# vin2803/scalable-hw-agnostic-inference

Hardware: AMD Instinct MI355X
Metric: SD2.1 512x512 images/sec (50 DDIM steps, CFG 7.5) (higher is better)
Workload: dtype bf16; 1 GPU; model=stabilityai/stable-diffusion-2-1 (UNet2DCondition 865M + OpenCLIP-H text + VAE), global_batch=32, per_gpu_batch=32, seq_len=77, resolution=512x512, inference_steps=50, scheduler=DDIM, parallelism=dp1, hip_graphs=True

## Files before the change

csrc/bindings.cpp:

```cpp
#include <ATen/ATen.h>
#include <c10/hip/HIPStream.h>
#include <torch/library.h>

#include <cmath>
#include <cstdio>
#include <cstdlib>
#include <mutex>
#include <string>
#include <unordered_map>
#include <algorithm>
#include <vector>

#include "kernels/launchers.h"

using at::Tensor;
using c10::optional;

namespace {

#define SHAI_CHECK(cond, ...) TORCH_CHECK(cond, "shai: ", __VA_ARGS__)

hipStream_t stream() { return c10::hip::getCurrentHIPStream().stream(); }

int g_halo_mode = -1;
// ... 1772 lines not shown
  if (bias.has_value()) {
    check_bf16(*bias, "bias");
    SHAI_CHECK(bias->numel() == g.N, "gemm_lnout bias [N]");
    g.bias = cptr(*bias);
  }
  for (const optional<Tensor>* t : {&gamma, &beta})
    if (t->has_value()) {
      check_bf16(**t, "gamma/beta");
      SHAI_CHECK((*t)->numel() == g.N, "gemm_lnout gamma / beta [N]");
    }
  if (!shai::gemm_ws_lnout_supported(g)) return false;
  shai::launch_gemm_ws_lnout(g, mptr(c2), optr(gamma), optr(beta), (float)eps, stream());
  return true;
}

void gemm_f8(const Tensor& a8, const Tensor& w8, const Tensor& a_scale, const Tensor& w_scale, const Tensor& c,
             const optional<Tensor>& bias, const optional<Tensor>& residual, double res_alpha, int64_t act, bool glu,
             int64_t cfg) {
  SHAI_CHECK(a8.is_cuda() && a8.scalar_type() == at::kFloat8_e4m3fn && a8.dim() == 2 && a8.stride(1) == 1,
             "gemm_f8: a8 must be float8_e4m3fn [M, K] with unit column stride");
  SHAI_CHECK(w8.is_cuda() && w8.scalar_type() == at::kFloat8_e4m3fn && w8.dim() == 2 && w8.is_contiguous(),
             "gemm_f8: w8 must be a contiguous float8_e4m3fn [N, K]");
  check_f32(a_scale, "a_scale");
  check_f32(w_scale, "w_scale");
  check_bf16(c, "c");
  const long M = a8.size(0), K = a8.size(1), N = w8.size(0);
  SHAI_CHECK(w8.size(1) == K && a_scale.numel() == M && w_scale.numel() == N, "gemm_f8 shapes");
  SHAI_CHECK(c.dim() == 2 && c.size(0) == M && c.size(1) == (glu ? N / 2 : N) && c.stride(1) == 1, "gemm_f8: c shape");
  shai::GemmArgs g{};
  g.M = (int)M;
// ... 67 lines not shown
  m.def("bias_act(Tensor x, Tensor? bias, Tensor? residual, Tensor(a!) out, int act, float alpha) -> ()");
  m.def("rope(Tensor(a!) x, Tensor positions, Tensor cos, Tensor sin, int rot_dim, bool neox) -> ()");
  m.def("rope_pairs(Tensor(a!) x, Tensor cos, Tensor sin) -> ()");
  m.def("sample(Tensor logits, Tensor temps, Tensor top_k, Tensor top_p, Tensor uniforms, Tensor(a!) out) -> ()");
  m.def("rope_qkv_cache(Tensor(a!) qkv, Tensor positions, Tensor cos, Tensor sin, Tensor(b!) k_cache, Tensor(c!) v_cache, Tensor slots, int H, int Hkv, float k_scale=1.0, float v_scale=1.0) -> ()");
  m.def("sched_step(Tensor model_out, Tensor(a!) latents, bool cfg, float guidance, int pred_type, float a_t, float a_prev, float dt) -> ()");
  m.def("sched_step_rows(Tensor model_out, Tensor(a!) latents, bool cfg, float guidance, int pred_type, Tensor rows_params) -> ()");
  m.def("softmax_(Tensor(a!) x, float scale) -> ()");
  m.def("embedding(Tensor ids, Tensor table, Tensor(a!) out) -> ()");
  m.def("token_feedback(Tensor(a!) ids, Tensor rowmap, Tensor prev) -> ()");
  m.def("decode_attn_rope(Tensor qkv, Tensor(a!) k_cache, Tensor(b!) v_cache, Tensor(c!) o, Tensor block_table, "
        "Tensor ctx_lens, Tensor positions, Tensor cos, Tensor sin, Tensor slots, Tensor(d!) ws, int h, int hk, "
        "int num_splits, float scale, Tensor? qkv_ws=None, int qkv_kg=0, int qkv_k=0, float qkv_eps=-1.0, float k_scale=1.0, float v_scale=1.0) -> ()");
  m.def("gemm_partials(Tensor a, Tensor w, float rms_eps) -> Tensor");
  m.def("gemm_lnout(Tensor a, Tensor w, Tensor(a!) c, Tensor(b!) c2, Tensor? bias, Tensor residual, float res_alpha, Tensor? gamma, Tensor? beta, float eps, int res_rows=0) -> bool");
  m.def("gemm_tuning() -> str[]", &gemm_tuning);
  m.def("gemm_tuning_export() -> str[]", &gemm_tuning_export);
  m.def("gemm_tuning_import(str[] entries) -> int", &gemm_tuning_import);
  m.def("set_halo_conv(int mode, int waves=-1) -> int", &set_halo_conv);
  m.def("set_flash128x2(int mode) -> int", [](int64_t mode) -> int64_t { return shai::set_flash128x2((int)mode); });
  m.def("set_decode_wb(int mode) -> int", [](int64_t mode) -> int64_t { return shai::set_decode_wb((int)mode); });
}

TORCH_LIBRARY_IMPL(shai, CUDA, m) {
  m.impl("rmsnorm", &rmsnorm);
  m.impl("layernorm", &layernorm);
  m.impl("groupnorm_stats", &groupnorm_stats);
  m.impl("groupnorm_from_partials", &groupnorm_from_partials);
  m.impl("col_partials", &col_partials);
  m.impl("row_moments", &row_moments);
  m.impl("groupnorm_apply", &groupnorm_apply);
  m.impl("gemm", &gemm);
  m.impl("dequant_fp8", &dequant_fp8);
  m.impl("dequant_mxfp4", &dequant_mxfp4);
  m.impl("gemm_f8", &gemm_f8);
  m.impl("gemm_lnout", &gemm_lnout);
  m.impl("quant_rows_fp8", &quant_rows_fp8);
  m.impl("layernorm_mod", &layernorm_mod);
  m.impl("qk_norm_rope", &qk_norm_rope);
  m.impl("conv2d", &conv2d);
  m.impl("flash_attn", &flash_attn);
  m.impl("paged_attn_varlen", &paged_attn_varlen);
  m.impl("decode_attn", &decode_attn);
  m.impl("kv_write", &kv_write);
  m.impl("kv_dequant_blocks", &kv_dequant_blocks);
  m.impl("gated_act", &gated_act);
  m.impl("bias_act", &bias_act);
  m.impl("rope", &rope);
  m.impl("rope_pairs", &rope_pairs);
  m.impl("sample", &sample);
  m.impl("rope_qkv_cache", &rope_qkv_cache);
// ... 9 lines not shown
```

csrc/build.py:

```python
#!/usr/bin/env python3
from __future__ import annotations

import argparse
import os
import shutil
import subprocess
import sys
import sysconfig

ROOT = os.path.dirname(os.path.dirname(os.path.abspath(__file__)))
CSRC = os.path.join(ROOT, "csrc")
PKG = os.path.join(ROOT, "scalable-hw-agnostic-inference_amd")
OUT = os.path.join(PKG, "_native")
BUILD = os.path.join(ROOT, "build", "native")
OUT_DEBUG = os.path.join(PKG, "_native_debug")
BUILD_DEBUG = os.path.join(ROOT, "build", "native_debug")
ARCH = os.environ.get("PYTORCH_ROCM_ARCH", "gfx950")
ROCM = os.environ.get("ROCM_PATH", "/opt/rocm")

KERNEL_SRCS = ["kernels/norm.hip", "kernels/gemm.hip", "kernels/gemm_lds.hip", "kernels/gemm_8ph.hip", "kernels/gemm_w4.hip", "kernels/gemm_ws.hip", "kernels/conv_halo.hip", "kernels/attention.hip", "kernels/attention2.hip", "kernels/attention3.hip", "kernels/elementwise.hip", "kernels/dit.hip",
               "kernels/sampling.hip", "kernels/gemv.hip", "kernels/gemv2.hip", "kernels/gemv_fp4.hip",
               "kernels/gemm_f8.hip", "kernels/attention_kv8.hip", "kernels/gemm_fp4.hip"]
NO_SCRATCH = {"kernels/attention.hip": "decode_attn_kernelINS_5KvFp8",
              "kernels/attention_kv8.hip": "flash_fwd_kernelINS_5KvFp8",
              "kernels/gemm_fp4.hip": "gemm_fp4_kernel"}
EXTRA_KFLAGS = {"kernels/attention3.hip": "-mllvm -amdgpu-mfma-vgpr-form -fno-slp-vectorize",
                "kernels/attention2.hip": "-mllvm -amdgpu-mfma-vgpr-form -fno-slp-vectorize",
                "kernels/gemm_w4.hip": "-mllvm -pragma-unroll-threshold=100000",
                "kernels/gemm_ws.hip": "-mllvm -pragma-unroll-threshold=100000 -fno-slp-vectorize",
                "kernels/conv_halo.hip": "-mllvm -pragma-unroll-threshold=100000 -fno-slp-vectorize"}
BINDING_SRCS = ["bindings.cpp", "test_probes.cpp"]
RUNTIME_SRCS = ["runtime/block_manager.cpp", "runtime/scheduler.cpp"]
COMM_SRCS = ["comm/p2p_allreduce.hip"]


def torch_paths():
    import torch
    from torch.utils import cpp_extension as ce
    inc = ce.include_paths(device_type="cuda") if "device_type" in ce.include_paths.__code__.co_varnames else ce.include_paths(True)
    lib = os.path.join(os.path.dirname(torch.__file__), "lib")
    abi = int(torch._C._GLIBCXX_USE_CXX11_ABI)
    return inc, lib, abi


def write_ninja(path: str, out: str = OUT, build_dir: str = BUILD, debug: bool = False) -> dict:
# ... 157 lines not shown
```

csrc/kernels/launchers.h:

```cpp
#pragma once
#include <hip/hip_runtime.h>
#include <stdint.h>

namespace shai {
typedef uint16_t bf16_t;

struct RowNormArgs {
  const bf16_t* x;
  const bf16_t* residual;
  const bf16_t* w;
  const bf16_t* b;
  bf16_t* out;
  bf16_t* residual_out;
  int rows, D;
  long x_stride, out_stride;
  float eps;
  float w_offset;
  int rows_per_w;
  long w_stride;
};
void launch_rmsnorm(const RowNormArgs& a, hipStream_t s);
void launch_layernorm(const RowNormArgs& a, hipStream_t s);

struct GroupNormArgs {
// ... 104 lines not shown
void launch_gemm(const GemmArgs& a, hipStream_t s);
void launch_gemm2(const GemmArgs& a, float* ws, hipStream_t s);
size_t gemm2_workspace_bytes(const GemmArgs& a);
void gemm2_plan(const GemmArgs& a, int* cfg, int* splits);
void launch_gemm2_cfg(const GemmArgs& a, float* ws, int cfg, int splits, hipStream_t s);
int gemm2_num_cfgs();
bool gemm2_cfg_supported(const GemmArgs& a, int cfg);
bool gemm2_cfg_splittable(int cfg);
bool gemm_w4_supported(const GemmArgs& a);
void launch_gemm_w4(const GemmArgs& a, int bn, hipStream_t s);
bool gemm_ws_supported(const GemmArgs& a);
void launch_gemm_ws(const GemmArgs& a, hipStream_t s);
bool gemm_ws_lnout_supported(const GemmArgs& a);
void launch_gemm_ws_lnout(const GemmArgs& a, bf16_t* C2, const bf16_t* gamma, const bf16_t* beta, float eps,
                          hipStream_t s);
bool conv_halo_supported(const GemmArgs& a);
void launch_conv_halo(const GemmArgs& a, hipStream_t s, int waves);
bool gemm2_cfg_candidate(int cfg);
void launch_splitk_epilogue(const GemmArgs& a, const float* ws, int splits, hipStream_t s);
bool gemm4_supported(const GemmArgs& a);
bool gemm4_stats_ok(const GemmArgs& a, int bn);
void launch_gemm4(const GemmArgs& a, float* ws, int splits, int bn, hipStream_t s, bool persist = false);
bool skinny_supported(const GemmArgs& a);
int skinny_kgroups(const GemmArgs& a);
int skinny_max_kgroups(const GemmArgs& a);
size_t skinny_workspace_bytes(const GemmArgs& a);
size_t skinny_workspace_bytes_kg(const GemmArgs& a, int kg);
void launch_skinny(const GemmArgs& a, float* ws, hipStream_t s);
void launch_skinny_kg(const GemmArgs& a, float* ws, int kg, hipStream_t s, bool fixup = false, bool fold = true);
unsigned* skinny_ticket_slice(hipStream_t s, int ntiles);
// ... 101 lines not shown
```

scalable-hw-agnostic-inference_amd/models/unet2d.py:

```python
from __future__ import annotations

import os
from dataclasses import dataclass, field
from typing import List, Optional, Tuple

import torch
import torch.nn as nn

from .. import ops
from .attention import CrossAttention, FusedSelfAttention, merge_linear_keys
from .layers import Conv2d, GLULinear, GroupNorm, LayerNorm, Linear, _wkey, timestep_embedding

MERGE_PROJ_OUT = os.environ.get("SHAI_MERGE_PROJ_OUT", "1") != "0"
GN_FOLD_PROJ_IN = os.environ.get("SHAI_GN_FOLD_PROJ_IN", "1") != "0"

NORM_HANDOFF = os.environ.get("SHAI_NORM_HANDOFF", "1") != "0"
FUSED_GN_CONV = os.environ.get("SHAI_FUSED_GN_CONV", "1") != "0"
CFG_SHARED = os.environ.get("SHAI_CFG_SHARED", "1") != "0"
CFG_SHARED_MIN_ROWS = int(os.environ.get("SHAI_CFG_SHARED_MIN_ROWS", "8192"))


@dataclass
class UNetConfig:
    in_channels: int = 4
# ... 73 lines not shown
class BasicTransformerBlock(nn.Module):
    def __init__(self, dim: int, heads: int, ctx_dim: int):
        super().__init__()
        self.norm1 = LayerNorm(dim)
        self.attn1 = FusedSelfAttention(dim, heads, qkv_bias=False)
        self.norm2 = LayerNorm(dim)
        self.attn2 = CrossAttention(dim, ctx_dim, heads)
        self.norm3 = LayerNorm(dim)
        self.ff = FeedForward(dim)

    def forward(self, x, ctx_kv, shared: bool = False):
        x = self.attn1(self.norm1(x), residual=x)
        x = self.attn2(self.norm2(x), ctx_kv, residual=x, shared=shared)
        return self.ff(self.norm3(x), residual=x)

    def forward_folded(self, x, ctx_kv, mr, next_eps=None, defer_down: bool = False, shared: bool = False):
        B, T, C = x.shape
        a1 = self.attn1
        w, b, s = a1.qkv.folded(self.norm1)
        q, k, v = a1.split(ops.linear(x, w, b, row_affine=(mr, s)))
        o = ops.attention(q, k, v)
        a2 = self.attn2
        H, hd = a2.heads, a2.head_dim
        lnout = x.is_cuda and ops.lnout_supported(B * T, C, a1.heads * a1.head_dim)
        if lnout:
            n2, n3 = self.norm2, self.norm3
            x, xn = ops.linear_lnout(o.view(B, T, a1.heads * a1.head_dim), a1.out.weight, a1.out.bias, x, n2.weight,
                                     n2.bias, n2.eps)
            q = a2.q(xn).view(B, T, H, hd)
        else:
            x, mr = a1.out.forward_stats(o.view(B, T, a1.heads * a1.head_dim), residual=x, stats="ln",
                                         eps=self.norm2.eps)
            w, b, s = a2.q.folded(self.norm2)
            q = ops.linear(x, w, b, row_affine=(mr, s)).view(B, T, H, hd)
        S = ctx_kv.shape[1]
        o = ops.attention(q, ctx_kv[..., : H * hd].view(ctx_kv.shape[0], S, H, hd),
                          ctx_kv[..., H * hd:].view(ctx_kv.shape[0], S, H, hd), q_batch_mod=B if shared else 0)
        rr = B * T if shared else 0
        B = o.shape[0]
        proj = self.ff.net[0].proj
        if lnout:
            x, xn = ops.linear_lnout(o.view(B, T, H * hd), a2.out.weight, a2.out.bias, x, self.norm3.weight,
                                     self.norm3.bias, self.norm3.eps, residual_rows=rr)
            h = ops.linear(xn, proj.weight, proj.bias, act=proj.act, glu=True)
        else:
            x, mr = a2.out.forward_stats(o.view(B, T, H * hd), residual=x, stats="ln", eps=self.norm3.eps,
                                         residual_rows=rr)
            w, b, s = proj.folded(self.norm3)
            h = ops.linear(x, w, b, act=proj.act, glu=True, row_affine=(mr, s))
        if defer_down:
            return h, x
        down = self.ff.net[2]
        if next_eps is None:
            return down(h, residual=x), None
        return down.forward_stats(h, residual=x, stats="ln", eps=next_eps)


class Transformer2DModel(nn.Module):
# ... 15 lines not shown
    def forward_parts(self, x, ctx_kv, xp=None, stats: bool = False, shared: bool = False):
        B, H, W, C = x.shape
        rr = B * H * W if shared else 0
        blocks = list(self.transformer_blocks)
        if ops.fold_profitable(B * H * W, C):
            if self._gn_fold_ok(x):
                h, mr = self._proj_in_gn_folded(x, xp, blocks[0].norm1.eps)
            else:
                h, mr = self.proj_in(self.norm(x, part=xp), stats="ln", eps=blocks[0].norm1.eps)
            h = h.view(B, H * W, C)
            if mr is None:
                mr = ops.row_moments(h, blocks[0].norm1.eps)
            merged = self._merged_out(x.is_cuda)
            for i, blk in enumerate(blocks):
                if i + 1 == len(blocks) and merged is not None:
                    ffh, hx = blk.forward_folded(h, ctx_kv, mr, None, defer_down=True, shared=shared and i == 0)
                    return self._out_merged(ffh, hx, x, merged, stats, rr)
                h, mr = blk.forward_folded(h, ctx_kv, mr, blocks[i + 1].norm1.eps if i + 1 < len(blocks) else None,
                                           shared=shared and i == 0)
        else:
            h = self.proj_in(self.norm(x, part=xp)).view(B, H * W, C)
            for i, blk in enumerate(blocks):
                h = blk(h, ctx_kv, shared=shared and i == 0)
        res = x.view(B, H * W, C)
        B = h.shape[0]
        if stats and ops.stats_supported(B * H * W, C, "gn", H * W):
            out, op = self.proj_out.forward_stats(h, residual=res, stats="gn", residual_rows=rr)
            return out.view(B, H, W, C), op
        return self.proj_out(h, residual=res, residual_rows=rr).view(B, H, W, C), None

    def _gn_fold_ok(self, x) -> bool:
# ... 16 lines not shown
        if down.in_features % 64 or po.in_features % 64:
            return None
        key = tuple(_wkey(t) for t in (down.weight, down.bias, po.weight, po.bias))
        cached = getattr(self, "_po_merged", None)
        if cached is None or cached[0] != key:
            if cuda and torch.cuda.is_current_stream_capturing():
                return None
            wpo = po.weight.float()
            w = torch.cat([wpo @ down.weight.float(), wpo], 1).to(po.weight.dtype).contiguous()
            b = po.bias.float() if po.bias is not None else torch.zeros(po.out_features, device=wpo.device)
            if down.bias is not None:
                b = b + wpo @ down.bias.float()
            cached = (key, (w, b.to(po.weight.dtype)))
            self._po_merged = cached
        return cached[1]

    def _out_merged(self, ffh, hx, x, merged, stats, residual_rows: int = 0):
        _, H, W, C = x.shape
        B = hx.shape[0]
        w, b = merged
        f = ffh.reshape(B, H, W, ffh.shape[-1])
        kw = {"stats": "gn"} if stats and ops.stats_supported(B * H * W, C, "gn", H * W) else {}
        r = ops.conv2d(f, w, b, 1, 1, x2=hx.reshape(B, H, W, C), residual=x, residual_rows=residual_rows, **kw)
        return r if kw else (r, None)


class Downsample2D(nn.Module):
    def __init__(self, ch):
        super().__init__()
        self.conv = Conv2d(ch, ch, 3, stride=2, padding=1)
# ... 195 lines not shown
```

scalable-hw-agnostic-inference_amd/ops/__init__.py:

```python
from __future__ import annotations

import math
import os
from dataclasses import dataclass
from typing import List, Optional, Sequence, Tuple

import torch

from .. import native
from . import reference as ref
from .reference import (ACT_GELU, ACT_GELU_TANH, ACT_NONE, ACT_QUICK_GELU, ACT_RELU, ACT_SILU, act_id, mxfp4_pack,
                        mxfp4_unpack, quantize_mxfp4, pack_conv_weight, pack_up2_phase_weight, unpack_conv_weight)

__all__ = [
    "rmsnorm", "layernorm", "groupnorm_stats", "groupnorm_apply", "groupnorm", "linear", "conv2d", "attention",
    "paged_attention", "decode_attention", "kv_write", "rope", "rope_pairs", "gated_act", "bias_act", "sched_step",
    "softmax_", "embedding", "token_feedback", "decode_attention_rope", "decode_attention_rope_qkv", "gemm_partials", "quantize_fp8_rows", "dequant_fp8", "quantize_mxfp4", "dequant_mxfp4", "mxfp4_pack", "mxfp4_unpack", "is_mxfp4", "quant_rows_fp8", "gemm_f8", "pack_conv_weight", "pack_up2_phase_weight", "linear_wslices", "unpack_conv_weight", "act_id", "ACT_NONE", "ACT_SILU", "ACT_GELU",
    "ACT_GELU_TANH", "ACT_QUICK_GELU", "ACT_RELU", "decode_splits", "set_decode_wb",
    "paged_attention_varlen", "rope_qkv_cache", "quantize_kv_fp8", "dequant_kv_fp8", "kv_dequant_blocks",
    "plan_kv_scratch", "build_kv_rounds", "KVRound", "FP8_KV_DTYPE", "resolve_kv_prefill", "KV_PREFILL_ROUTES",
]


def _gpu(t: torch.Tensor) -> bool:
    return t.is_cuda


def _K():
    return native.ops()


def _i32(t: Optional[torch.Tensor]):
# ... 271 lines not shown
    x2 = x.reshape(-1, K) if (x.dim() == 2 or x.is_contiguous()) else x.contiguous().reshape(-1, K)
    r2 = residual.reshape(-1, N)
    y = torch.empty(x2.shape[0], N, dtype=x.dtype, device=x.device)
    y2 = torch.empty_like(y)
    if LNOUT and _K().gemm_lnout(x2, w, y, y2, bias, r2, 1.0, gamma, beta, float(eps), int(residual_rows)):
        return y.view(*x.shape[:-1], N), y2.view(*x.shape[:-1], N)
    y = linear(x, w, bias, residual=residual, residual_rows=residual_rows)
    return y, layernorm(y, gamma, beta, eps)[0]


LNOUT = os.environ.get("SHAI_LNOUT", "1") != "0"


def lnout_supported(rows: int, n: int, k: int) -> bool:
    return LNOUT and n == 320 and k == 320


def fold_layernorm(w: torch.Tensor, bias: Optional[torch.Tensor], gamma: Optional[torch.Tensor],
                   beta: Optional[torch.Tensor]):
    wf = w.float()
    w2 = (wf * gamma.float()[None, :]).to(w.dtype) if gamma is not None else w
    b2 = bias.float() if bias is not None else torch.zeros(w.shape[0], dtype=torch.float32, device=w.device)
    if beta is not None:
        b2 = b2 + wf @ beta.float()
    return w2.contiguous(), b2.to(w.dtype), w2.float().sum(1).contiguous()


def row_moments(x: torch.Tensor, eps: float) -> torch.Tensor:
    x2 = x.reshape(-1, x.shape[-1])
    if not _gpu(x):
# ... 516 lines not shown
```

scalable-hw-agnostic-inference_amd/ops/reference.py:

```python
from __future__ import annotations

import math

import torch
import torch.nn.functional as F

ACT_NONE, ACT_SILU, ACT_GELU, ACT_GELU_TANH, ACT_QUICK_GELU, ACT_RELU = range(6)
ACT_IDS = {"none": ACT_NONE, None: ACT_NONE, "silu": ACT_SILU, "gelu": ACT_GELU, "gelu_tanh": ACT_GELU_TANH,
           "gelu_pytorch_tanh": ACT_GELU_TANH, "gelu_new": ACT_GELU_TANH, "quick_gelu": ACT_QUICK_GELU,
           "relu": ACT_RELU, "swish": ACT_SILU}


def act_id(act) -> int:
    if isinstance(act, int):
        return act
    return ACT_IDS[act]


def apply_act(x: torch.Tensor, act) -> torch.Tensor:
    a = act_id(act)
    if a == ACT_SILU:
        return F.silu(x)
    if a == ACT_GELU:
        return F.gelu(x)
# ... 100 lines not shown
        y = (mr[:, 1:2] * (y2 - mr[:, 0:1] * s.float()[None, :])).reshape(y.shape)
    y = y * alpha
    if bias is not None:
        y = y + bias.float()
    if glu:
        val, gate = y[..., 0::2], y[..., 1::2]
        y = val * apply_act(gate, act)
    else:
        y = apply_act(y, act)
    if residual is not None:
        r = residual.float()
        if residual_rows:
            r = wrap_rows(r, y.numel() // y.shape[-1], y.shape[-1]).reshape(y.shape)
        y = y + res_alpha * r
    return y.to(x.dtype)


MXFP4_GROUP = 32
MXFP4_VALUES = (0.0, 0.5, 1.0, 1.5, 2.0, 3.0, 4.0, 6.0)


def mxfp4_pack(codes: torch.Tensor, scale_bytes: torch.Tensor):
    N, K2 = codes.shape
    G = scale_bytes.shape[1]
    assert codes.dtype == torch.uint8 and scale_bytes.dtype == torch.uint8 and scale_bytes.shape[0] == N
    assert K2 * 2 == G * MXFP4_GROUP, "one scale per 32 codes"
    steps = (G + 3) // 4
    sb = torch.full((N, steps * 4), 127, dtype=torch.uint8, device=codes.device)
    sb[:, :G] = scale_bytes
    tiled = sb.view(N, steps, 4).permute(1, 0, 2).contiguous()
# ... 390 lines not shown
```

Baseline: 12.28 images/s.

## Fuse GEGLU feed-forward up-projection with merged down/proj_out GEMM in one kernel

Result: no change. 12.30 images/s (median of 2 runs) (+0.1%).

```diff
diff --git a/csrc/bindings.cpp b/csrc/bindings.cpp
--- a/csrc/bindings.cpp
+++ b/csrc/bindings.cpp
@@ -1810,6 +1810,60 @@
   return true;
 }
 
+bool ff_fused(const Tensor& xn, const Tensor& hx, const Tensor& xres, const Tensor& w1, const optional<Tensor>& b1,
+              const Tensor& wm, const optional<Tensor>& bm, const Tensor& out, const optional<Tensor>& part,
+              int64_t res_rows, int64_t max_wgs) {
+  check_rows(xn, "xn");
+  check_rows(hx, "hx");
+  check_rows(xres, "xres");
+  check_rows(w1, "w1");
+  check_rows(wm, "wm");
+  check_bf16(out, "out");
+  if (xn.dim() != 2 || hx.dim() != 2 || xres.dim() != 2 || w1.dim() != 2 || wm.dim() != 2 || out.dim() != 2)
+    return false;
+  shai::FfArgs g{};
+  g.M = (int)xn.size(0);
+  g.C = (int)xn.size(1);
+  g.F = (int)(w1.size(0) / 2);
+  SHAI_CHECK(w1.size(0) == 2 * (int64_t)g.F && w1.size(1) == g.C && wm.size(0) == g.C && wm.size(1) == g.F + g.C,
+             "ff_fused: weights must be w1 [2F, C] and wm [C, F + C]");
+  SHAI_CHECK(hx.size(0) == g.M && hx.size(1) == g.C && out.size(0) == g.M && out.size(1) == g.C &&
+                 xres.size(1) == g.C && xres.size(0) == (res_rows > 0 ? res_rows : (int64_t)g.M),
+             "ff_fused: activation / output / residual shape mismatch");
+  if (res_rows > 0 && res_rows != g.M) g.res_rows = (int)res_rows;
+  g.xn = cptr(xn);
+  g.hx = cptr(hx);
+  g.xres = cptr(xres);
+  g.W1 = cptr(w1);
+  g.Wm = cptr(wm);
+  g.out = mptr(out);
+  g.ldxn = xn.stride(0);
+  g.ldhx = hx.stride(0);
+  g.ldres = xres.stride(0);
+  g.ldw1 = w1.stride(0);
+  g.ldwm = wm.stride(0);
+  g.ldo = out.stride(0);
+  g.max_wgs = (int)max_wgs;
+  if (b1.has_value()) {
+    check_bf16(*b1, "b1");
+    SHAI_CHECK(b1->numel() == 2 * (int64_t)g.F && b1->is_contiguous(), "ff_fused: b1 [2F]");
+    g.b1 = cptr(*b1);
+  }
+  if (bm.has_value()) {
+    check_bf16(*bm, "bm");
+    SHAI_CHECK(bm->numel() == g.C && bm->is_contiguous(), "ff_fused: bm [C]");
+    g.bm = cptr(*bm);
+  }
+  if (part.has_value()) {
+    check_f32(*part, "part");
+    SHAI_CHECK(part->numel() == (int64_t)((g.M + 127) / 128) * g.C * 2, "ff_fused: part [ceil(M / 128), C, 2]");
+    g.col_part = part->data_ptr<float>();
+  }
+  if (!shai::gemm_ff_supported(g)) return false;
+  shai::launch_gemm_ff(g, stream());
+  return true;
+}
+
 void gemm_f8(const Tensor& a8, const Tensor& w8, const Tensor& a_scale, const Tensor& w_scale, const Tensor& c,
              const optional<Tensor>& bias, const optional<Tensor>& residual, double res_alpha, int64_t act, bool glu,
              int64_t cfg) {
@@ -1907,6 +1961,8 @@
         "int num_splits, float scale, Tensor? qkv_ws=None, int qkv_kg=0, int qkv_k=0, float qkv_eps=-1.0, float k_scale=1.0, float v_scale=1.0) -> ()");
   m.def("gemm_partials(Tensor a, Tensor w, float rms_eps) -> Tensor");
   m.def("gemm_lnout(Tensor a, Tensor w, Tensor(a!) c, Tensor(b!) c2, Tensor? bias, Tensor residual, float res_alpha, Tensor? gamma, Tensor? beta, float eps, int res_rows=0) -> bool");
+  m.def("ff_fused(Tensor xn, Tensor hx, Tensor xres, Tensor w1, Tensor? b1, Tensor wm, Tensor? bm, Tensor(a!) out, Tensor(b!)? part, int res_rows=0, int max_wgs=0) -> bool");
+  m.def("ff_fused_set_ablation(int mode) -> ()", [](int64_t mode) { shai::gemm_ff_set_ablation((int)mode); });
   m.def("gemm_tuning() -> str[]", &gemm_tuning);
   m.def("gemm_tuning_export() -> str[]", &gemm_tuning_export);
   m.def("gemm_tuning_import(str[] entries) -> int", &gemm_tuning_import);
@@ -1928,6 +1984,7 @@
   m.impl("dequant_mxfp4", &dequant_mxfp4);
   m.impl("gemm_f8", &gemm_f8);
   m.impl("gemm_lnout", &gemm_lnout);
+  m.impl("ff_fused", &ff_fused);
   m.impl("quant_rows_fp8", &quant_rows_fp8);
   m.impl("layernorm_mod", &layernorm_mod);
   m.impl("qk_norm_rope", &qk_norm_rope);
diff --git a/csrc/build.py b/csrc/build.py
--- a/csrc/build.py
+++ b/csrc/build.py
@@ -18,17 +18,20 @@
 ARCH = os.environ.get("PYTORCH_ROCM_ARCH", "gfx950")
 ROCM = os.environ.get("ROCM_PATH", "/opt/rocm")
 
-KERNEL_SRCS = ["kernels/norm.hip", "kernels/gemm.hip", "kernels/gemm_lds.hip", "kernels/gemm_8ph.hip", "kernels/gemm_w4.hip", "kernels/gemm_ws.hip", "kernels/conv_halo.hip", "kernels/attention.hip", "kernels/attention2.hip", "kernels/attention3.hip", "kernels/elementwise.hip", "kernels/dit.hip",
+KERNEL_SRCS = ["kernels/norm.hip", "kernels/gemm.hip", "kernels/gemm_lds.hip", "kernels/gemm_8ph.hip", "kernels/gemm_w4.hip", "kernels/gemm_ws.hip", "kernels/gemm_ff.hip", "kernels/conv_halo.hip", "kernels/attention.hip", "kernels/attention2.hip", "kernels/attention3.hip", "kernels/elementwise.hip", "kernels/dit.hip",
                "kernels/sampling.hip", "kernels/gemv.hip", "kernels/gemv2.hip", "kernels/gemv_fp4.hip",
                "kernels/gemm_f8.hip", "kernels/attention_kv8.hip", "kernels/gemm_fp4.hip"]
 NO_SCRATCH = {"kernels/attention.hip": "decode_attn_kernelINS_5KvFp8",
               "kernels/attention_kv8.hip": "flash_fwd_kernelINS_5KvFp8",
-              "kernels/gemm_fp4.hip": "gemm_fp4_kernel"}
+              "kernels/gemm_fp4.hip": "gemm_fp4_kernel",
+              "kernels/gemm_ff.hip": "gemm_ff_kernel"}
 EXTRA_KFLAGS = {"kernels/attention3.hip": "-mllvm -amdgpu-mfma-vgpr-form -fno-slp-vectorize",
                 "kernels/attention2.hip": "-mllvm -amdgpu-mfma-vgpr-form -fno-slp-vectorize",
                 "kernels/gemm_w4.hip": "-mllvm -pragma-unroll-threshold=100000",
                 "kernels/gemm_ws.hip": "-mllvm -pragma-unroll-threshold=100000 -fno-slp-vectorize",
-                "kernels/conv_halo.hip": "-mllvm -pragma-unroll-threshold=100000 -fno-slp-vectorize"}
+                "kernels/conv_halo.hip": "-mllvm -pragma-unroll-threshold=100000 -fno-slp-vectorize",
+                "kernels/gemm_ff.hip": ("-mllvm -pragma-unroll-threshold=100000 -fno-slp-vectorize "
+                                        "-mllvm -amdgpu-mfma-vgpr-form")}
 BINDING_SRCS = ["bindings.cpp", "test_probes.cpp"]
 RUNTIME_SRCS = ["runtime/block_manager.cpp", "runtime/scheduler.cpp"]
 COMM_SRCS = ["comm/p2p_allreduce.hip"]
diff --git a/csrc/kernels/gemm_ff.hip b/csrc/kernels/gemm_ff.hip
--- /dev/null
+++ b/csrc/kernels/gemm_ff.hip
@@ -0,0 +1,466 @@
+#include "common.h"
+#include "launchers.h"
+
+#include <algorithm>
+#include <type_traits>
+
+namespace shai {
+
+typedef __bf16 ffbf16x8 __attribute__((ext_vector_type(8)));
+typedef float fff2 __attribute__((ext_vector_type(2)));
+typedef __bf16 ffbf2 __attribute__((ext_vector_type(2)));
+typedef __attribute__((address_space(3))) void ff_lds_void;
+
+constexpr int FF_C = 320, FF_F = 1280, FF_BM = 128;
+constexpr int FF_HC = 32;
+constexpr int FF_NCH = FF_F / FF_HC;
+constexpr int FF_PIECE = 20480;
+constexpr int FF_RING = 7;
+constexpr int FF_AHEAD = FF_RING - 1;
+constexpr int FF_DMA = 5;
+constexpr int FF_B1 = FF_RING * FF_PIECE;
+constexpr int FF_BMO = FF_B1 + 2 * FF_F * 2;
+constexpr int FF_PART = FF_BMO + FF_C * 4;
+constexpr int FF_LDS = FF_PART + 4 * FF_C * 2 * 4;
+constexpr uint32_t FF_OOB = 0x80000000u;
+constexpr int FF_NLD = 20;
+static_assert(FF_LDS <= 160 * 1024, "LDS");
+
+__device__ __forceinline__ __amdgpu_buffer_rsrc_t ff_rsrc(const void* base, long bytes) {
+  return __builtin_amdgcn_make_buffer_rsrc(const_cast<void*>(base), (short)0, (int)(bytes < 0x7fffffffL ? bytes : 0x7fffffffL),
+                                           0x00020000);
+}
+
+__device__ __forceinline__ uint32_t ff_pk(float a, float b) {
+  const fff2 v = {a, b};
+  return __builtin_bit_cast(uint32_t, __builtin_convertvector(v, ffbf2));
+}
+
+__device__ __forceinline__ float ff_row16_sum(float x) {
+  x += __builtin_bit_cast(float, __builtin_amdgcn_update_dpp(0, __builtin_bit_cast(int, x), 0xB1, 0xf, 0xf, true));
+  x += __builtin_bit_cast(float, __builtin_amdgcn_update_dpp(0, __builtin_bit_cast(int, x), 0x4E, 0xf, 0xf, true));
+  x += __builtin_bit_cast(float, __builtin_amdgcn_update_dpp(0, __builtin_bit_cast(int, x), 0x141, 0xf, 0xf, true));
+  x += __builtin_bit_cast(float, __builtin_amdgcn_update_dpp(0, __builtin_bit_cast(int, x), 0x140, 0xf, 0xf, true));
+  return x;
+}
+
+template <bool STATS, int ABL>
+__global__ void __launch_bounds__(256, 1) gemm_ff_kernel(const FfArgs p) {
+  extern __shared__ __attribute__((aligned(16))) char ff_smem[];
+  bf16_t* s_b1 = reinterpret_cast<bf16_t*>(ff_smem + FF_B1);
+  float* s_bm = reinterpret_cast<float*>(ff_smem + FF_BMO);
+  float* s_part = reinterpret_cast<float*>(ff_smem + FF_PART);
+
+  const int tid = threadIdx.x, lane = tid & 63;
+  const int wid = __builtin_amdgcn_readfirstlane(tid >> 6);
+  const int fr = lane & 15, fq = lane >> 4;
+  const int tiles = (p.M + FF_BM - 1) / FF_BM;
+
+  for (int i = tid; i < 2 * FF_F; i += 256) s_b1[i] = p.b1 ? p.b1[i] : (bf16_t)0;
+  for (int i = tid; i < FF_C; i += 256) s_bm[i] = p.bm ? bf2f(p.bm[i]) : 0.f;
+  __syncthreads();
+
+  const long w1_bytes = (long)2 * FF_F * p.ldw1 * 2, wm_bytes = (long)FF_C * p.ldwm * 2;
+  const long xn_bytes = ((long)(p.M - 1) * p.ldxn + FF_C) * 2, hx_bytes = ((long)(p.M - 1) * p.ldhx + FF_C) * 2;
+  const int rrows = p.res_rows > 0 ? p.res_rows : p.M;
+  const long xr_bytes = ((long)(rrows - 1) * p.ldres + FF_C) * 2;
+  const __amdgpu_buffer_rsrc_t rW1 = ff_rsrc(p.W1, w1_bytes), rWm = ff_rsrc(p.Wm, wm_bytes);
+  const __amdgpu_buffer_rsrc_t rXn = ff_rsrc(p.xn, xn_bytes), rHx = ff_rsrc(p.hx, hx_bytes);
+  const __amdgpu_buffer_rsrc_t rXr = ff_rsrc(p.xres, xr_bytes);
+
+  uint32_t off1l[2];
+#pragma unroll
+  for (int e = 0; e < 2; ++e) {
+    const int Rp = 8 * e + (lane >> 3), r = Rp & 15;
+    off1l[e] = (uint32_t)(((16 * (r >> 2) + (r & 3)) * FF_C + (((lane & 7) ^ ((Rp >> 1) & 7)) << 3)) * 2);
+  }
+  auto off1u = [&](int i) {
+    const int q = wid * FF_DMA + i, kt = q >> 2, b = (q & 3) >> 1;
+    return (uint32_t)((4 * b * FF_C + kt * 64) * 2);
+  };
+  uint32_t offml;
+  {
+    const int r = lane >> 2, sc = (lane & 3) ^ ((-(r >> 2)) & 3);
+    offml = (uint32_t)(((8 * (r >> 2) + (r & 3)) * (FF_F + FF_C) + sc * 8) * 2);
+  }
+  auto offmu = [&](int i) {
+    const int j = wid * FF_DMA + i;
+    return (uint32_t)((32 * (j >> 1) + 4 * (j & 1)) * (FF_F + FF_C) * 2);
+  };
+  struct Piece {
+    bool w1;
+    uint32_t so;
+  };
+  auto piece_w1 = [](int c, int h) { return Piece{true, (uint32_t)(c * 64 + h * 8) * (uint32_t)(FF_C * 2)}; };
+  auto piece_wm = [](int kcol) { return Piece{false, (uint32_t)kcol * 2u}; };
+  auto piece_of = [&](int g, int k) {
+    if (g < FF_NCH) return k < 2 ? piece_w1(g, k) : piece_wm(g >= 1 ? FF_HC * (g - 1) : 0);
+    const int idx = 3 * (g - FF_NCH) + k;
+    return piece_wm(idx == 0 ? FF_HC * (FF_NCH - 1) : idx <= 10 ? FF_F + 32 * (idx - 1) : 0);
+  };
+  auto dma_i = [&](const Piece pc, int slot, int i) {
+    if constexpr ((ABL & 4) != 0) return;
+    SHAI_DASSERT(slot >= 0 && slot < FF_RING && i >= 0 && i < FF_DMA);
+    char* dst = ff_smem + slot * FF_PIECE + (wid * FF_DMA + i) * 1024;
+    if (pc.w1) {
+      const uint32_t so = off1u(i) + pc.so;
+      SHAI_DASSERT_DMA(off1l[(wid * FF_DMA + i) & 1] + so, w1_bytes, FF_OOB);
+      __builtin_amdgcn_raw_ptr_buffer_load_lds(rW1, (ff_lds_void*)dst, 16, off1l[(wid * FF_DMA + i) & 1], so, 0, 0);
+    } else {
+      const uint32_t so = offmu(i) + pc.so;
+      SHAI_DASSERT_DMA(offml + so, wm_bytes, FF_OOB);
+      __builtin_amdgcn_raw_ptr_buffer_load_lds(rWm, (ff_lds_void*)dst, 16, offml, so, 0, 0);
+    }
+  };
+
+  const int w1rd = fr * 128, w1sw = (fr >> 1) & 7;
+  auto w1frag = [&](const char* piece, int b, int s) {
+    return *reinterpret_cast<const ffbf16x8*>(piece + (s >> 1) * 4096 + b * 2048 + w1rd +
+                                              (((4 * (s & 1) + fq) ^ w1sw) << 4));
+  };
+  const int wmrd = fr * 64 + ((fq ^ ((-(fr >> 2)) & 3)) << 4);
+  auto wmfrag = [&](const char* piece, int j) {
+    return *reinterpret_cast<const ffbf16x8*>(piece + j * 1024 + wmrd);
+  };
+
+  auto load_rows = [&](const __amdgpu_buffer_rsrc_t& rs, long ld, long r0, int rows, uint4_ (&x)[2][10], int s0,
+                       int s1) {
+#pragma unroll
+    for (int rb = 0; rb < 2; ++rb) {
+      const long row = r0 + 32 * wid + 16 * rb + fr;
+      const uint32_t off = row < rows ? (uint32_t)((row * ld + 8 * fq) * 2) : FF_OOB;
+#pragma unroll
+      for (int s = 0; s < 10; ++s)
+        if (s >= s0 && s < s1)
+          x[rb][s] = __builtin_bit_cast(uint4_, __builtin_amdgcn_raw_buffer_load_b128(rs, (int)(off + 64u * s), 0, 0));
+    }
+  };
+
+  float4_ out[2][20];
+  uint4_ xf[2][10], hf[2][10], rf[2][10];
+  float4_ accA[2][4], accB[2][4];
+
+  auto gemm1 = [&](const char* piece, int h, float4_ (&acc)[2][4], auto&& pre, auto&& between) {
+    ffbf16x8 w[3][2];
+#pragma unroll
+    for (int s = 0; s < 2; ++s)
+#pragma unroll
+      for (int b = 0; b < 2; ++b) w[s][b] = w1frag(piece, b, s);
+#pragma unroll
+    for (int s = 0; s < 10; ++s) {
+      pre(s);
+      if (s + 2 < 10) {
+#pragma unroll
+        for (int b = 0; b < 2; ++b) w[(s + 2) % 3][b] = w1frag(piece, b, s + 2);
+      }
+      __builtin_amdgcn_sched_barrier(0);
+#pragma unroll
+      for (int b = 0; b < 2; ++b)
+#pragma unroll
+        for (int rb = 0; rb < 2; ++rb)
+          acc[rb][2 * h + b] = __builtin_amdgcn_mfma_f32_16x16x32_bf16(
+              w[s % 3][b], __builtin_bit_cast(ffbf16x8, xf[rb][s]),
+              s == 0 ? float4_{0.f, 0.f, 0.f, 0.f} : acc[rb][2 * h + b], 0, 0, 0);
+      if (between(s)) {
+#pragma unroll
+        for (int i = 0; i < 4; ++i) {
+          __builtin_amdgcn_sched_group_barrier(0x008, 1, 0);
+          __builtin_amdgcn_sched_group_barrier(0x002, 5, 0);
+        }
+      }
+      __builtin_amdgcn_sched_barrier(0);
+    }
+  };
+  auto glu_bias = [&](int c, int u) {
+    const uint2_ b = *reinterpret_cast<const uint2_*>(s_b1 + 64 * c + 16 * fq + 4 * (u & 3));
+    return float4_{bf2f(b[0] & 0xffff), bf2f(b[0] >> 16), bf2f(b[1] & 0xffff), bf2f(b[1] >> 16)};
+  };
+  auto glu_half = [&](const float4_ (&acc)[2][4], const float4_ b, int x, float (&o)[2], uint32_t (&ff)[2][4]) {
+    const int u = x >> 1, e = x & 1, rb = u >> 2, jj = u & 3;
+    const float v = acc[rb][jj][2 * e] + b[2 * e], g = acc[rb][jj][2 * e + 1] + b[2 * e + 1];
+    if constexpr ((ABL & 2) != 0) o[e] = v * g;
+    else o[e] = v * gelu_erf_f(g);
+    if (e == 1) ff[rb][jj] = ff_pk(o[0], o[1]);
+  };
+  auto gemm2 = [&](const char* piece, const ffbf16x8 b0, const ffbf16x8 b1, auto&& pre) {
+    ffbf16x8 w[5];
+#pragma unroll
+    for (int j = 0; j < 4; ++j) w[j] = wmfrag(piece, j);
+#pragma unroll
+    for (int j = 0; j < 20; ++j) {
+      pre(j);
+      if (j + 4 < 20) w[(j + 4) % 5] = wmfrag(piece, j + 4);
+      __builtin_amdgcn_sched_barrier(0);
+      out[0][j] = __builtin_amdgcn_mfma_f32_16x16x32_bf16(w[j % 5], b0, out[0][j], 0, 0, 0);
+      out[1][j] = __builtin_amdgcn_mfma_f32_16x16x32_bf16(w[j % 5], b1, out[1][j], 0, 0, 0);
+    }
+    __builtin_amdgcn_sched_barrier(0);
+  };
+
+  int cs = 0;
+  auto sync = [&](auto extra) {
+    constexpr int N = (FF_AHEAD - 1) * FF_DMA + decltype(extra)::value;
+    if constexpr (SHAI_DEBUG) asm volatile("s_waitcnt vmcnt(0)" ::: "memory");
+    else asm volatile("s_waitcnt vmcnt(%0)" ::"n"(N > 63 ? 63 : N) : "memory");
+    asm volatile("s_waitcnt lgkmcnt(0)" ::: "memory");
+    __builtin_amdgcn_sched_barrier(0);
+    __builtin_amdgcn_s_barrier();
+    __builtin_amdgcn_sched_barrier(0);
+  };
+  auto next_slot = [&]() { cs = cs + 1 == FF_RING ? 0 : cs + 1; };
+  auto prev_slot = [&]() { return cs == 0 ? FF_RING - 1 : cs - 1; };
+  using E0 = std::integral_constant<int, 0>;
+  using E20 = std::integral_constant<int, FF_NLD>;
+  using E40 = std::integral_constant<int, 2 * FF_NLD>;
+
+  auto step_w1 = [&](auto extra, const Piece ahead, int c, int h, float4_ (&accN)[2][4], const float4_ (&accP)[2][4],
+                     bool prev, float4_ (&gb)[2], float (&o)[2], uint32_t (&ff)[2][4]) {
+    sync(extra);
+    const int ps = prev_slot();
+    const char* piece = ff_smem + cs * FF_PIECE;
+    if (prev) gb[0] = glu_bias(c - 1, 4 * h);
+    gemm1(
+        piece, h, accN,
+        [&](int s) {
+          if (s < FF_DMA) dma_i(ahead, ps, s);
+          const int nx = 8 * h + s + 1;
+          if (prev && s + 1 < 8 && nx % 2 == 0) gb[(nx >> 1) & 1] = glu_bias(c - 1, nx >> 1);
+        },
+        [&](int s) {
+          if (prev && s < 8) glu_half(accP, gb[((8 * h + s) >> 1) & 1], 8 * h + s, o, ff);
+          return prev && s < 8;
+        });
+    next_slot();
+  };
+  auto step_wm = [&](auto extra, const Piece ahead, const ffbf16x8 b0, const ffbf16x8 b1, auto&& mid) {
+    sync(extra);
+    const int ps = prev_slot();
+    const char* piece = ff_smem + cs * FF_PIECE;
+    mid();
+    gemm2(piece, b0, b1, [&](int j) {
+      if (j % 4 == 0) dma_i(ahead, ps, j / 4);
+    });
+    next_slot();
+  };
+  auto ffrag = [](const uint32_t (&ff)[2][4], int rb) {
+    return __builtin_bit_cast(ffbf16x8, uint4_{ff[rb][0], ff[rb][1], ff[rb][2], ff[rb][3]});
+  };
+  auto hfrag = [&](int rb, int t) { return __builtin_bit_cast(ffbf16x8, hf[rb][t]); };
+  auto step_idle = [&](auto extra, const Piece ahead) {
+    sync(extra);
+    const int ps = prev_slot();
+#pragma unroll
+    for (int i = 0; i < FF_DMA; ++i) dma_i(ahead, ps, i);
+    __builtin_amdgcn_sched_barrier(0);
+    next_slot();
+  };
+  auto group = [&](auto extra, int c, float4_ (&accN)[2][4], const float4_ (&accP)[2][4]) {
+    float4_ gb[2];
+    float o[2];
+    uint32_t ff[2][4];
+    step_w1(extra, piece_of(c + 2, 0), c, 0, accN, accP, true, gb, o, ff);
+    step_w1(extra, piece_of(c + 2, 1), c, 1, accN, accP, true, gb, o, ff);
+    step_wm(extra, piece_of(c + 2, 2), ffrag(ff, 0), ffrag(ff, 1), [] {});
+  };
+
+#pragma unroll
+  for (int n = 0; n < FF_AHEAD; ++n)
+#pragma unroll
+    for (int i = 0; i < FF_DMA; ++i) dma_i(piece_of(n / 3, n % 3), n, i);
+  __builtin_amdgcn_sched_barrier(0);
+  load_rows(rXn, p.ldxn, (long)blockIdx.x * FF_BM, p.M, xf, 0, 10);
+  __builtin_amdgcn_sched_barrier(0);
+  bool counted = false, first = true;
+
+  for (int tile = blockIdx.x; tile < tiles; tile += gridDim.x) {
+    const long m0 = (long)tile * FF_BM;
+#pragma unroll
+    for (int rb = 0; rb < 2; ++rb)
+#pragma unroll
+      for (int j = 0; j < 20; ++j) out[rb][j] = float4_{0.f, 0.f, 0.f, 0.f};
+
+    {
+      float4_ gb[2];
+      float o[2];
+      uint32_t ff[2][4];
+      if (!first && counted) {
+        step_w1(E40{}, piece_of(2, 0), 0, 0, accA, accB, false, gb, o, ff);
+        step_w1(E40{}, piece_of(2, 1), 0, 1, accA, accB, false, gb, o, ff);
+        step_idle(E40{}, piece_of(2, 2));
+      } else {
+        step_w1(E20{}, piece_of(2, 0), 0, 0, accA, accB, false, gb, o, ff);
+        step_w1(E20{}, piece_of(2, 1), 0, 1, accA, accB, false, gb, o, ff);
+        step_idle(E20{}, piece_of(2, 2));
+      }
+      if (first || counted) group(E20{}, 1, accB, accA);
+      else group(E0{}, 1, accB, accA);
+      first = false;
+    }
+    for (int c = 2; c < 38; c += 2) {
+      group(E0{}, c, accA, accB);
+      group(E0{}, c + 1, accB, accA);
+    }
+    group(E0{}, 38, accA, accB);
+    {
+      float4_ gb[2];
+      float o[2];
+      uint32_t ff[2][4];
+      step_w1(E0{}, piece_of(41, 0), 39, 0, accB, accA, true, gb, o, ff);
+      load_rows(rHx, p.ldhx, m0, p.M, hf, 0, 3);
+      __builtin_amdgcn_sched_barrier(0);
+      step_w1(E0{}, piece_of(41, 1), 39, 1, accB, accA, true, gb, o, ff);
+      step_wm(E0{}, piece_of(41, 2), ffrag(ff, 0), ffrag(ff, 1), [] {});
+      load_rows(rXn, p.ldxn, m0 + (long)gridDim.x * FF_BM, p.M, xf, 0, 10);
+      __builtin_amdgcn_sched_barrier(0);
+    }
+    {
+      float o[2];
+      uint32_t ff[2][4];
+#pragma unroll
+      for (int x = 0; x < 16; ++x) glu_half(accB, glu_bias(FF_NCH - 1, x >> 1), x, o, ff);
+      step_wm(E20{}, piece_of(42, 0), ffrag(ff, 0), ffrag(ff, 1), [] {});
+    }
+    auto hx_next = [&](int t) {
+      load_rows(rHx, p.ldhx, m0, p.M, hf, t, t + 1);
+      __builtin_amdgcn_sched_barrier(0);
+    };
+    hx_next(3);
+    step_wm(E20{}, piece_of(42, 1), hfrag(0, 0), hfrag(1, 0), [] {});
+    hx_next(4);
+    step_wm(E20{}, piece_of(42, 2), hfrag(0, 1), hfrag(1, 1), [] {});
+    hx_next(5);
+    step_wm(E20{}, piece_of(43, 0), hfrag(0, 2), hfrag(1, 2), [] {});
+    hx_next(6);
+    step_wm(E20{}, piece_of(43, 1), hfrag(0, 3), hfrag(1, 3), [] {});
+    hx_next(7);
+    step_wm(E20{}, piece_of(43, 2), hfrag(0, 4), hfrag(1, 4), [] {});
+    hx_next(8);
+    step_wm(E0{}, piece_of(0, 0), hfrag(0, 5), hfrag(1, 5), [] {});
+    hx_next(9);
+    step_wm(E0{}, piece_of(0, 1), hfrag(0, 6), hfrag(1, 6), [] {});
+    step_wm(E0{}, piece_of(0, 2), hfrag(0, 7), hfrag(1, 7), [] {});
+    load_rows(rXr, p.ldres, p.res_rows > 0 ? m0 % p.res_rows : m0, rrows, rf, 0, 10);
+    __builtin_amdgcn_sched_barrier(0);
+    step_wm(E20{}, piece_of(1, 0), hfrag(0, 8), hfrag(1, 8), [] {});
+    step_wm(E20{}, piece_of(1, 1), hfrag(0, 9), hfrag(1, 9), [] {});
+    step_idle(E20{}, piece_of(1, 2));
+
+    const bool full = m0 + FF_BM <= p.M;
+#pragma unroll
+    for (int q = 0; q < 10; ++q) {
+      const int c0 = 32 * q + 8 * fq;
+      const float4_ b0 = *reinterpret_cast<const float4_*>(s_bm + c0);
+      const float4_ b1 = *reinterpret_cast<const float4_*>(s_bm + c0 + 4);
+      float cs[8], cq[8];
+#pragma unroll
+      for (int e = 0; e < 8; ++e) cs[e] = cq[e] = 0.f;
+#pragma unroll
+      for (int rb = 0; rb < 2; ++rb) {
+        const long m = m0 + 32 * wid + 16 * rb + fr;
+        const bool ok = m < p.M;
+        float r8[8], v[8];
+        unpack8(rf[rb][q], r8);
+#pragma unroll
+        for (int e = 0; e < 4; ++e) {
+          v[e] = (out[rb][2 * q][e] + b0[e]) + r8[e];
+          v[4 + e] = (out[rb][2 * q + 1][e] + b1[e]) + r8[4 + e];
+        }
+        uint4_ w;
+#pragma unroll
+        for (int e = 0; e < 4; ++e) w[e] = ff_pk(v[2 * e], v[2 * e + 1]);
+        if constexpr ((ABL & 1) != 0) {
+#pragma unroll
+          for (int e = 0; e < 4; ++e) asm volatile("" ::"v"(w[e]));
+        } else {
+          if (ok) *reinterpret_cast<uint4_*>(p.out + m * p.ldo + c0) = w;
+        }
+        if constexpr (STATS) {
+          float f[8];
+          unpack8(w, f);
+#pragma unroll
+          for (int e = 0; e < 8; ++e) {
+            const float x = ok ? f[e] : 0.f;
+            cs[e] += x;
+            cq[e] = fmaf(x, x, cq[e]);
+          }
+        }
+      }
+      if constexpr (STATS) {
+#pragma unroll
+        for (int e = 0; e < 8; ++e) {
+          cs[e] = ff_row16_sum(cs[e]);
+          cq[e] = ff_row16_sum(cq[e]);
+        }
+        if (fr == 0) {
+          float4_* dst = reinterpret_cast<float4_*>(s_part + (wid * FF_C + c0) * 2);
+#pragma unroll
+          for (int e = 0; e < 4; ++e) dst[e] = float4_{cs[2 * e], cq[2 * e], cs[2 * e + 1], cq[2 * e + 1]};
+        }
+      }
+    }
+    if constexpr (STATS) {
+      asm volatile("s_waitcnt lgkmcnt(0)" ::: "memory");
+      __builtin_amdgcn_sched_barrier(0);
+      __builtin_amdgcn_s_barrier();
+      __builtin_amdgcn_sched_barrier(0);
+      if (tid < FF_C / 2) {
+        float4_ t = *reinterpret_cast<const float4_*>(s_part + 4 * tid);
+#pragma unroll
+        for (int w = 1; w < 4; ++w) t += *reinterpret_cast<const float4_*>(s_part + w * FF_C * 2 + 4 * tid);
+        *reinterpret_cast<float4_*>(p.col_part + ((long)tile * FF_C) * 2 + 4 * tid) = t;
+      }
+      counted = false;
+    } else {
+      counted = full && !(ABL & 1);
+    }
+  }
+  asm volatile("s_waitcnt vmcnt(0)" ::: "memory");
+}
+
+bool gemm_ff_supported(const FfArgs& a) {
+  if (a.C != FF_C || a.F != FF_F || a.M <= 0) return false;
+  if (!a.xn || !a.hx || !a.xres || !a.W1 || !a.Wm || !a.out) return false;
+  if (a.ldw1 != FF_C || a.ldwm != FF_F + FF_C) return false;
+  if (a.ldxn % 8 || a.ldhx % 8 || a.ldres % 8 || a.ldo % 8) return false;
+  if (a.ldxn < FF_C || a.ldhx < FF_C || a.ldres < FF_C || a.ldo < FF_C) return false;
+  const auto al = [](const void* q) { return ((uintptr_t)q & 15) == 0; };
+  if (!al(a.xn) || !al(a.hx) || !al(a.xres) || !al(a.W1) || !al(a.Wm) || !al(a.out)) return false;
+  if (a.col_part && !al(a.col_part)) return false;
+  if (a.res_rows < 0 || (a.res_rows > 0 && (a.res_rows % FF_BM != 0 || a.M % a.res_rows != 0))) return false;
+  const long lim = 0x7fffffffL;
+  const long rr = a.res_rows > 0 ? a.res_rows : a.M;
+  if ((long)a.M * a.ldxn * 2 >= lim || (long)a.M * a.ldhx * 2 >= lim || rr * a.ldres * 2 >= lim) return false;
+  return true;
+}
+
+static int ff_cus() {
+  static int w = [] {
+    int dev = 0, cus = 0;
+    if (hipGetDevice(&dev) != hipSuccess ||
+        hipDeviceGetAttribute(&cus, hipDeviceAttributeMultiprocessorCount, dev) != hipSuccess || cus < 1)
+      cus = 256;
+    return cus;
+  }();
+  return w;
+}
+
+static int ff_ablation = 0;
+void gemm_ff_set_ablation(int a) { ff_ablation = a; }
+
+void launch_gemm_ff(const FfArgs& a, hipStream_t s) {
+  const int tiles = (a.M + FF_BM - 1) / FF_BM;
+  int grid = std::min(ff_cus(), tiles);
+  if (a.max_wgs > 0) grid = std::min(grid, a.max_wgs);
+#ifdef SHAI_GEMM_LAB
+  switch (ff_ablation) {
+    case 1: gemm_ff_kernel<false, 1><<<grid, 256, FF_LDS, s>>>(a); return;
+    case 2: gemm_ff_kernel<false, 2><<<grid, 256, FF_LDS, s>>>(a); return;
+    case 4: gemm_ff_kernel<false, 4><<<grid, 256, FF_LDS, s>>>(a); return;
+    default: break;
+  }
+#endif
+  if (a.col_part) gemm_ff_kernel<true, 0><<<grid, 256, FF_LDS, s>>>(a);
+  else gemm_ff_kernel<false, 0><<<grid, 256, FF_LDS, s>>>(a);
+}
+
+}
diff --git a/csrc/kernels/launchers.h b/csrc/kernels/launchers.h
--- a/csrc/kernels/launchers.h
+++ b/csrc/kernels/launchers.h
@@ -142,6 +142,24 @@
 bool gemm_ws_lnout_supported(const GemmArgs& a);
 void launch_gemm_ws_lnout(const GemmArgs& a, bf16_t* C2, const bf16_t* gamma, const bf16_t* beta, float eps,
                           hipStream_t s);
+struct FfArgs {
+  const bf16_t* xn;
+  const bf16_t* hx;
+  const bf16_t* xres;
+  const bf16_t* W1;
+  const bf16_t* b1;
+  const bf16_t* Wm;
+  const bf16_t* bm;
+  bf16_t* out;
+  float* col_part;
+  int M, C, F;
+  int res_rows;
+  long ldxn, ldhx, ldres, ldw1, ldwm, ldo;
+  int max_wgs;
+};
+bool gemm_ff_supported(const FfArgs& a);
+void launch_gemm_ff(const FfArgs& a, hipStream_t s);
+void gemm_ff_set_ablation(int a);
 bool conv_halo_supported(const GemmArgs& a);
 void launch_conv_halo(const GemmArgs& a, hipStream_t s, int waves);
 bool gemm2_cfg_candidate(int cfg);
diff --git a/scalable-hw-agnostic-inference_amd/models/unet2d.py b/scalable-hw-agnostic-inference_amd/models/unet2d.py
--- a/scalable-hw-agnostic-inference_amd/models/unet2d.py
+++ b/scalable-hw-agnostic-inference_amd/models/unet2d.py
@@ -111,7 +111,8 @@
         x = self.attn2(self.norm2(x), ctx_kv, residual=x, shared=shared)
         return self.ff(self.norm3(x), residual=x)
 
-    def forward_folded(self, x, ctx_kv, mr, next_eps=None, defer_down: bool = False, shared: bool = False):
+    def forward_folded(self, x, ctx_kv, mr, next_eps=None, defer_down: bool = False, shared: bool = False,
+                       fuse_ff: bool = False):
         B, T, C = x.shape
         a1 = self.attn1
         w, b, s = a1.qkv.folded(self.norm1)
@@ -139,6 +140,8 @@
         if lnout:
             x, xn = ops.linear_lnout(o.view(B, T, H * hd), a2.out.weight, a2.out.bias, x, self.norm3.weight,
                                      self.norm3.bias, self.norm3.eps, residual_rows=rr)
+            if defer_down and fuse_ff:
+                return None, x, xn
             h = ops.linear(xn, proj.weight, proj.bias, act=proj.act, glu=True)
         else:
             x, mr = a2.out.forward_stats(o.view(B, T, H * hd), residual=x, stats="ln", eps=self.norm3.eps,
@@ -184,7 +187,16 @@
             merged = self._merged_out(x.is_cuda)
             for i, blk in enumerate(blocks):
                 if i + 1 == len(blocks) and merged is not None:
-                    ffh, hx = blk.forward_folded(h, ctx_kv, mr, None, defer_down=True, shared=shared and i == 0)
+                    sh = shared and i == 0
+                    proj = blk.ff.net[0].proj
+                    fuse = (x.is_cuda and proj.act == "gelu"
+                            and ops.ff_fused_wanted((ctx_kv.shape[0] if sh else h.shape[0]) * H * W, C, proj.hidden))
+                    ffh, hx, *xn = blk.forward_folded(h, ctx_kv, mr, None, defer_down=True, shared=sh, fuse_ff=fuse)
+                    if xn:
+                        r = self._out_fused(xn[0], hx, x, proj, merged, stats, rr)
+                        if r is not None:
+                            return r
+                        ffh = ops.linear(xn[0], proj.weight, proj.bias, act=proj.act, glu=True)
                     return self._out_merged(ffh, hx, x, merged, stats, rr)
                 h, mr = blk.forward_folded(h, ctx_kv, mr, blocks[i + 1].norm1.eps if i + 1 < len(blocks) else None,
                                            shared=shared and i == 0)
@@ -231,6 +243,17 @@
             cached = (key, (w, b.to(po.weight.dtype)))
             self._po_merged = cached
         return cached[1]
+
+    def _out_fused(self, xn, hx, x, proj, merged, stats, residual_rows: int = 0):
+        _, H, W, C = x.shape
+        B = hx.shape[0]
+        w, b = merged
+        want = bool(stats) and ops.stats_supported(B * H * W, C, "gn", H * W)
+        r = ops.ff_fused(xn, hx, x, proj.weight, proj.bias, w, b, residual_rows=residual_rows, stats=want)
+        if r is None:
+            return None
+        out, part = r if want else (r, None)
+        return out.view(B, H, W, C), part
 
     def _out_merged(self, ffh, hx, x, merged, stats, residual_rows: int = 0):
         _, H, W, C = x.shape
diff --git a/scalable-hw-agnostic-inference_amd/ops/__init__.py b/scalable-hw-agnostic-inference_amd/ops/__init__.py
--- a/scalable-hw-agnostic-inference_amd/ops/__init__.py
+++ b/scalable-hw-agnostic-inference_amd/ops/__init__.py
@@ -15,7 +15,7 @@
 __all__ = [
     "rmsnorm", "layernorm", "groupnorm_stats", "groupnorm_apply", "groupnorm", "linear", "conv2d", "attention",
     "paged_attention", "decode_attention", "kv_write", "rope", "rope_pairs", "gated_act", "bias_act", "sched_step",
-    "softmax_", "embedding", "token_feedback", "decode_attention_rope", "decode_attention_rope_qkv", "gemm_partials", "quantize_fp8_rows", "dequant_fp8", "quantize_mxfp4", "dequant_mxfp4", "mxfp4_pack", "mxfp4_unpack", "is_mxfp4", "quant_rows_fp8", "gemm_f8", "pack_conv_weight", "pack_up2_phase_weight", "linear_wslices", "unpack_conv_weight", "act_id", "ACT_NONE", "ACT_SILU", "ACT_GELU",
+    "softmax_", "embedding", "token_feedback", "decode_attention_rope", "decode_attention_rope_qkv", "gemm_partials", "quantize_fp8_rows", "dequant_fp8", "quantize_mxfp4", "dequant_mxfp4", "mxfp4_pack", "mxfp4_unpack", "is_mxfp4", "quant_rows_fp8", "gemm_f8", "pack_conv_weight", "pack_up2_phase_weight", "linear_wslices", "ff_fused", "ff_fused_wanted", "unpack_conv_weight", "act_id", "ACT_NONE", "ACT_SILU", "ACT_GELU",
     "ACT_GELU_TANH", "ACT_QUICK_GELU", "ACT_RELU", "decode_splits", "set_decode_wb",
     "paged_attention_varlen", "rope_qkv_cache", "quantize_kv_fp8", "dequant_kv_fp8", "kv_dequant_blocks",
     "plan_kv_scratch", "build_kv_rounds", "KVRound", "FP8_KV_DTYPE", "resolve_kv_prefill", "KV_PREFILL_ROUTES",
@@ -317,6 +317,34 @@
 
 def lnout_supported(rows: int, n: int, k: int) -> bool:
     return LNOUT and n == 320 and k == 320
+
+
+FF_FUSED = os.environ.get("SHAI_FF_FUSED", "")
+FF_FUSED_MIN_ROWS = int(os.environ.get("SHAI_FF_FUSED_MIN_ROWS", "32768"))
+FF_FUSED_CALLS = 0
+
+
+def ff_fused_wanted(rows: int, c: int, f: int) -> bool:
+    if FF_FUSED == "0" or c != 320 or f != 1280:
+        return False
+    return FF_FUSED == "1" or rows >= FF_FUSED_MIN_ROWS
+
+
+def ff_fused(xn: torch.Tensor, hx: torch.Tensor, xres: torch.Tensor, w1: torch.Tensor, b1, wm: torch.Tensor, bm,
+             residual_rows: int = 0, stats: bool = False, max_wgs: int = 0):
+    global FF_FUSED_CALLS
+    C = xn.shape[-1]
+    xn2, hx2, xr2 = xn.reshape(-1, C), hx.reshape(-1, C), xres.reshape(-1, C)
+    if not _gpu(xn):
+        out = ref.ff_fused(xn2, hx2, xr2, w1, b1, wm, bm, residual_rows)
+        return (out, ref.col_partials(out)) if stats else out
+    M = xn2.shape[0]
+    out = torch.empty(M, C, dtype=xn.dtype, device=xn.device)
+    part = torch.empty((M + 127) // 128, C, 2, dtype=torch.float32, device=xn.device) if stats else None
+    if not _K().ff_fused(xn2, hx2, xr2, w1, b1, wm, bm, out, part, int(residual_rows), int(max_wgs)):
+        return None
+    FF_FUSED_CALLS += 1
+    return (out, part) if stats else out
 
 
 def fold_layernorm(w: torch.Tensor, bias: Optional[torch.Tensor], gamma: Optional[torch.Tensor],
diff --git a/scalable-hw-agnostic-inference_amd/ops/reference.py b/scalable-hw-agnostic-inference_amd/ops/reference.py
--- a/scalable-hw-agnostic-inference_amd/ops/reference.py
+++ b/scalable-hw-agnostic-inference_amd/ops/reference.py
@@ -138,6 +138,13 @@
             r = wrap_rows(r, y.numel() // y.shape[-1], y.shape[-1]).reshape(y.shape)
         y = y + res_alpha * r
     return y.to(x.dtype)
+
+
+def ff_fused(xn, hx, xres, w1, b1, wm, bm, residual_rows=0):
+    M, C = xn.shape
+    f = linear(xn, w1, b1, act="gelu", glu=True)
+    return conv2d(f.view(1, M, 1, -1), wm, bm, 1, 1, x2=hx.view(1, M, 1, C), residual=xres.view(1, -1, 1, C),
+                  residual_rows=residual_rows).view(M, C)
 
 
 MXFP4_GROUP = 32
```
